# KevynUtopia/Frequency-Aware-Inverse-Consistent-OCTA-Super-Resolution

Hardware: AMD Instinct MI355X
Metric: train-step images/sec (G+D fwd+bwd) on 256x256 OCTA (higher is better)
Workload: dtype f32 (tensors and accumulators fp32; the convolutions' operands enter the matrix cores as f16x2 pairs: hi = f16(x 2^k), lo = f16(x 2^k - hi), k from the tensor's largest magnitude; 3 v_mfma_f32_32x32x16_f16 per product) on every map >= 24 wide with >= 16 channels; narrow maps, 1-channel stems / head

## Files before the change

frequency-aware-inverse-consistent-octa-super-resolution_amd/_lib.py:

```python
import ctypes
import os

import torch

_HERE = os.path.dirname(os.path.abspath(__file__))
LIB_PATH = os.environ.get("FAOCTASR_LIB") or os.path.join(_HERE, "libfaoctasr.so")

_P, _I, _L, _F = ctypes.c_void_p, ctypes.c_int, ctypes.c_long, ctypes.c_float
_SIG = {
    "version": (_I, ""),
    "last_error": (ctypes.c_char_p, ""),
    "last_route": (_I, ""),
    "conv_wpack_floats": (_L, "iiiiiiii"),
    "conv_pack_job": (_L, "p l i pp iiiiiiiii i i i"),
    "conv_pack_run": (_I, "p i l p"),
    "conv_pack_scales": (_I, "p i p"),
    "absmax_bits": (_I, "p l p p"),
    "conv_set_scales": (_I, "pp"),
    "conv_needs_scales": (_I, "i iiiiiiiii i i"),
    "out_absmax": (_I, "p"),
    "conv_set_workspace": (_I, "p l"),
    "conv_set_residual": (_I, "p"),
    "conv_wgrad_workspace_floats": (_L, "iiiii"),
    "conv_gather_workspace_floats": (_L, "i iiiiiiiii i i"),
    "conv2d_fwd": (_I, "pppp iiiiiiiii i i f p i i p"),
    "conv2d_dgrad": (_I, "ppp iiiiiiiii p i i p"),
    "conv2d_wgrad": (_I, "ppp iiiiiiiii i i i p"),
    "conv_transpose2d_fwd": (_I, "pppp iiiiiiiii i i f p i i p"),
    "conv_transpose2d_dgrad": (_I, "ppp iiiiiiiii i p i i p"),
    "conv_transpose2d_wgrad": (_I, "ppp iiiiiiiii i i i p"),
    "reflect_pad_bwd": (_I, "pp iiii p"),
    "channel_sum": (_I, "pp iii i p"),
    "bn_workspace_floats": (_L, "i"),
    "batchnorm_train_fwd": (_I, "ppppppppp iii ff i f p p"),
    "batchnorm_train_bwd": (_I, "ppppppppppp iii i f i p p"),
    "batchnorm_eval_fwd": (_I, "pppppp iii f i f p"),
    "batchnorm_eval_bwd": (_I, "ppppp iii f i f p"),
    "instancenorm_fwd": (_I, "pppppp iii f i f p p"),
    "instancenorm_bwd": (_I, "pppppppppp iii i f p p"),
    "act_fwd": (_I, "pp l i f p"),
    "act_bwd": (_I, "ppp l i f p"),
    "cat2_act_fwd": (_I, "ppp iiii i f p"),
    "cat2_act_bwd": (_I, "pppp iiii i f p"),
    "axpby": (_I, "ppp l ff p"),
    "haar_dwt2d_fwd": (_I, "ppp l ii p"),
    "haar_dwt2d_bwd": (_I, "ppp l ii p"),
    "haar_dfront_fwd": (_I, "pp iii i p"),
    "haar_dfront_bwd": (_I, "pp iii i p"),
    "sgemm_batched": (_I, "ppp iii iii lll i p"),
    "freq_mix_fwd": (_I, "ppppp l p"),
    "freq_mix_bwd": (_I, "pppppppp l p"),
    "ssim_fwd": (_I, "ppp iiii p"),
    "ssim_bwd": (_I, "ppp i f pp iiii p"),
    "dft_tables": (_I, "p i p"),
    "phase_loss_workspace_floats": (_L, "iiii"),
    "phase_loss_fwd": (_I, "pppp f ppp iiii p"),
    "phase_loss_bwd": (_I, "ppp f ppp iiii p"),
    "ffl_workspace_floats": (_L, "iiii"),
    "ffl_fwd": (_I, "pppp f ii ppp iiii p"),
    "ffl_bwd": (_I, "pppp f i ppp iiii p"),
    "mi_workspace_floats": (_L, "iiii i"),
    "mi_fwd": (_I, "pp ppp iiii i ffff ii p"),
    "mi_bwd": (_I, "ppp p pp iiii i fff i p"),
    "tv_loss_workspace_floats": (_L, "iiii"),
    "tv_loss_fwd": (_I, "ppp iiii f p"),
    "tv_loss_bwd": (_I, "ppp iiii f p"),
    "dwt2d_analysis": (_I, "ppp l ii ppi ppi i p"),
    "dwt2d_synthesis": (_I, "ppp l iiii ppi ppi i p"),
    "dwt1d_fused_max": (_L, ""),
    "dwt1d_analysis": (_I, "p lll pp l i p i pp i i i p"),
    "dwt1d_synthesis": (_I, "p lll pp l p i i pp i i i p"),
    "swt2d_analysis": (_I, "p l p l ii ppi ppi i i f p"),
    "swt2d_adjoint": (_I, "pp l p l i l ii ppi ppi i i f p"),
    "dtcwt_fwd_j1": (_I, "p lll pp llllll i l iii pi pi i p"),
    "dtcwt_fwd_j2": (_I, "p lll pp llllll i l iii pppp i p"),
    "dtcwt_inv_j1": (_I, "p lll p llllll p l iii pi pi i p"),
    "dtcwt_inv_j2": (_I, "p lll p llllll p l iii pppp i p"),
    "scat_fwd_j1": (_I, "p lll p ll i p lll p i ff l iii pi pi i p"),
    "scat_fwd_j2": (_I, "p lll p ll p lll p i ff l iii pppp i p"),
    "scat_bwd_j1": (_I, "p ll i p lll p p l iii pi pi i p"),
    "scat_bwd_j2": (_I, "p ll p lll p p l iii pppp i p"),
    "dtcwt_fwd_j1_bp": (_I, "p lll pp llllll i l iii pi pi pi i p"),
    "dtcwt_fwd_j2_bp": (_I, "p lll pp llllll i l iii pppppp i p"),
    "dtcwt_inv_j1_bp": (_I, "p lll p llllll p l iii pi pi pi i p"),
    "dtcwt_inv_j2_bp": (_I, "p lll p llllll p l iii pppppp i p"),
    "scat_fwd_j1_bp": (_I, "p lll p ll i p lll p i ff l iii pi pi pi i p"),
    "scat_fwd_j2_bp": (_I, "p lll p ll p lll p i ff l iii pppppp i p"),
    "scat_bwd_j1_bp": (_I, "p ll i p lll p p l iii pi pi pi i p"),
    "scat_bwd_j2_bp": (_I, "p ll p lll p p l iii pppppp i p"),
    "dtcwt_loss_workspace_floats": (_L, "l iii i"),
    "dtcwt_loss_fwd_j1": (_I, "p lll p lll pp pp p ff l iii pi pi i p"),
    "dtcwt_loss_fwd_j2": (_I, "p lll p lll pp pp p ff l iii pppp i p"),
    "dtcwt_loss_final": (_I, "p pp i p p"),
    "cwssim_workspace_floats": (_L, "l iii"),
    "cwssim_index": (_I, "pp pp p l iii f p"),
    "cwssim_grad": (_I, "pp pp pp p l l iii p"),
    "cwssim_final": (_I, "p l l iii pp p"),
    "msssim_workspace_floats": (_L, "l iii"),
    "msssim_scale_fwd": (_I, "pp pp p l iii i ff p"),
    "msssim_final": (_I, "p ll iii p i ppp p"),
    "msssim_scale_bwd": (_I, "pp p p i pp pp ll iii i ff p"),
    "loss_workspace_floats": (_L, ""),
    "loss_fwd": (_I, "ppp l i f p p"),
    "loss_bwd": (_I, "pppp l i f i p"),
    "mean_mix_fwd": (_I, "ppp iii ff p"),
    "mean_mix_bwd": (_I, "ppp iii ff p"),
    "adamw_step": (_I, "pppp l fffff i f p"),
    "adamw_step_dev": (_I, "pppp l p p"),
    "prep_crop_resize": (_I, "pppp iiiii ff p"),
    "fill": (_I, "p l f p"),
    "circulant_lowpass": (_I, "p i f p"),
    "eval_workspace_bytes": (_L, "ii"),
    "eval_metrics": (_I, "pppp iii f i p"),
    "bn_fold": (_I, "pppppp f pp i l i l p"),
# ... 92 lines not shown
```

frequency-aware-inverse-consistent-octa-super-resolution_amd/build.py:

```python
import os
import subprocess
from concurrent.futures import ThreadPoolExecutor

HERE = os.path.dirname(os.path.abspath(__file__))
ROOT = os.path.dirname(HERE)
SOURCES = ["igemm.hip", "igemm_patch.hip", "igemm_bf16x3.hip", "igemm_wino.hip", "igemm_nm.hip", "igemm_nm_x2.hip", "wgrad_patch.hip", "wgrad_s1.hip", "wgrad_x3.hip", "conv_m1.hip", "pointwise.hip", "norm.hip", "sgemm.hip",
           "ssim.hip", "spectral.hip", "mi.hip", "tv.hip", "dwt.hip", "dwt1d.hip", "swt.hip", "dtcwt.hip", "scat.hip", "dtcwt_loss.hip", "cwssim.hip", "msssim.hip", "eval.hip", "comm.hip", "conv_pack.hip", "conv_stem.hip"]
HEADERS = [os.path.join(HERE, "csrc", "common.h"), os.path.join(HERE, "csrc", "igemm_geom.h"), os.path.join(HERE, "csrc", "pack_bodies.h"), os.path.join(HERE, "csrc", "split16.h"), os.path.join(HERE, "csrc", "dtcwt_dev.h"),
           os.path.join(HERE, "csrc", "filterbank_dev.h"), os.path.join(HERE, "csrc", "ssim_window.h"),
           os.path.join(ROOT, "include", "faoctasr.h")]
FILE_FLAGS = {"ssim.hip": ["-fno-slp-vectorize"]}
LIB = os.path.join(HERE, "libfaoctasr.so")
OBJ_DIR = os.path.join(ROOT, "build", "obj")


def _flags():
    extra = os.environ.get("FAOCTASR_HIPCC_FLAGS", "").split()
    return ["-O3", "--offload-arch=gfx950", "-fPIC", "-std=c++17"] + extra + ["-I" + os.path.join(ROOT, "include"), "-I" + os.path.join(HERE, "csrc")]


def _stale(target, deps):
    if not os.path.exists(target):
        return True
    t = os.path.getmtime(target)
    return any(os.path.getmtime(d) > t for d in deps if os.path.exists(d))


def needs_build():
    srcs = [os.path.join(HERE, "csrc", s) for s in SOURCES]
    return _stale(LIB, srcs + HEADERS)


def build(force=False, verbose=False):
    hipcc = os.environ.get("HIPCC", "/opt/rocm/bin/hipcc")
    os.makedirs(OBJ_DIR, exist_ok=True)
    tag = "_".join(os.environ.get("FAOCTASR_HIPCC_FLAGS", "").split()).replace("/", "_").replace("=", "-")
    jobs, objs = [], []
    for s in SOURCES:
        src = os.path.join(HERE, "csrc", s)
        obj = os.path.join(OBJ_DIR, s + (("." + tag) if tag else "") + ".o")
        objs.append(obj)
        if force or _stale(obj, [src] + HEADERS):
            jobs.append((s, [hipcc] + _flags() + FILE_FLAGS.get(s, []) + ["-c", src, "-o", obj]))

    def run(job):
        name, cmd = job
        r = subprocess.run(cmd, stdout=subprocess.PIPE, stderr=subprocess.STDOUT, text=True)
        if r.returncode != 0:
            raise RuntimeError("hipcc failed on %s:\n%s\n%s" % (name, " ".join(cmd), r.stdout))
        return name

    if jobs:
        with ThreadPoolExecutor(max_workers=min(6, len(jobs))) as ex:
            done = list(ex.map(run, jobs))
        if verbose:
            print("compiled for gfx950:", " ".join(done))
    if jobs or force or _stale(LIB, objs):
        cmd = [hipcc, "--offload-arch=gfx950", "-fPIC", "-shared"] + objs + ["-ldl", "-o", LIB + ".tmp"]
        r = subprocess.run(cmd, stdout=subprocess.PIPE, stderr=subprocess.STDOUT, text=True)
        if r.returncode != 0:
            raise RuntimeError("link failed:\n%s\n%s" % (" ".join(cmd), r.stdout))
        os.replace(LIB + ".tmp", LIB)
        if verbose:
            print("linked", LIB)
    elif verbose:
        print("up to date:", LIB)
    return LIB


if __name__ == "__main__":
    import sys
    print(build(force="--force" in sys.argv, verbose=True))
```

frequency-aware-inverse-consistent-octa-super-resolution_amd/csrc/pointwise.hip:

```cpp
#include <mutex>
#include <unordered_map>
#include "common.h"
#include "split16.h"

namespace faoctasr {

thread_local char g_err[512] = "";
char* err_buf() { return g_err; }
int get_route();
int fail(int code, const char* fmt, ...) {
    va_list ap;
    va_start(ap, fmt);
    vsnprintf(g_err, sizeof(g_err), fmt, ap);
    va_end(ap);
    return code;
}

thread_local int g_route = 0;
thread_local unsigned* g_out_absmax = nullptr;
unsigned* take_out_absmax() {
    unsigned* p = g_out_absmax;
    g_out_absmax = nullptr;
    return p;
}
// ... 378 lines not shown
    constexpr float A = -0.75f;
    const float x0 = t + 1.f, x1 = t, x2 = 1.f - t, x3 = 2.f - t;
    c[0] = ((A * x0 - 5.f * A) * x0 + 8.f * A) * x0 - 4.f * A;
    c[1] = ((A + 2.f) * x1 - (A + 3.f)) * x1 * x1 + 1.f;
    c[2] = ((A + 2.f) * x2 - (A + 3.f)) * x2 * x2 + 1.f;
    c[3] = ((A * x3 - 5.f * A) * x3 + 8.f * A) * x3 - 4.f * A;
}

__global__ void prep_crop_resize_kernel(const unsigned char* __restrict__ img, const int* __restrict__ tops, const int* __restrict__ lefts,
                                        float* __restrict__ out, int N, int H, int W, int crop, int osz, float mean, float inv_std) {
    const long total = (long)N * osz * osz;
    const float scale = (float)crop / (float)osz;
    for (long i = (long)blockIdx.x * blockDim.x + threadIdx.x; i < total; i += (long)gridDim.x * blockDim.x) {
        const int ox = (int)(i % osz), oy = (int)((i / osz) % osz), n = (int)(i / ((long)osz * osz));
        const unsigned char* src = img + (long)n * H * W + (long)tops[n] * W + lefts[n];
        float v;
        if (osz == crop) {
            v = (float)src[(long)oy * W + ox] / 255.f;
        } else {
            const float sy = ((float)oy + 0.5f) * scale - 0.5f, sx = ((float)ox + 0.5f) * scale - 0.5f;
            const float fy = floorf(sy), fx = floorf(sx);
            float cy[4], cx[4];
            cubic_coeffs(sy - fy, cy);
            cubic_coeffs(sx - fx, cx);
            const int iy = (int)fy, ix = (int)fx;
            v = 0.f;
#pragma unroll
            for (int a = 0; a < 4; ++a) {
                int yy = iy - 1 + a;
                yy = yy < 0 ? 0 : (yy > crop - 1 ? crop - 1 : yy);
                float row = 0.f;
#pragma unroll
                for (int b = 0; b < 4; ++b) {
                    int xx = ix - 1 + b;
                    xx = xx < 0 ? 0 : (xx > crop - 1 ? crop - 1 : xx);
                    row += cx[b] * ((float)src[(long)yy * W + xx] / 255.f);
                }
                v += cy[a] * row;
            }
        }
        out[i] = (v - mean) * inv_std;
    }
}

__global__ __launch_bounds__(256) void absmax_bits_kernel(const float* __restrict__ x, long n, unsigned* __restrict__ slot) {
    typedef unsigned u32x4v __attribute__((ext_vector_type(4)));
    unsigned mx = 0;
    const long n4 = (reinterpret_cast<unsigned long>(x) & 15) ? 0 : n >> 2;
    const u32x4v* x4 = reinterpret_cast<const u32x4v*>(x);
    const long stride = (long)gridDim.x * 256;
    long i = (long)blockIdx.x * 256 + threadIdx.x;
    for (; i + 3 * stride < n4; i += 4 * stride) {
        const u32x4v v0 = x4[i], v1 = x4[i + stride], v2 = x4[i + 2 * stride], v3 = x4[i + 3 * stride];
#pragma unroll
        for (int j = 0; j < 4; ++j) {
            const unsigned a = v0[j] & 0x7fffffffu, b = v1[j] & 0x7fffffffu, c = v2[j] & 0x7fffffffu, d = v3[j] & 0x7fffffffu;
            const unsigned ab = a > b ? a : b, cd = c > d ? c : d;
            const unsigned m4 = ab > cd ? ab : cd;
            mx = m4 > mx ? m4 : mx;
        }
    }
    for (; i < n4; i += stride) {
        const u32x4v v = x4[i];
#pragma unroll
        for (int j = 0; j < 4; ++j) {
            const unsigned b = v[j] & 0x7fffffffu;
            mx = b > mx ? b : mx;
        }
    }
    for (long k = (n4 << 2) + (long)blockIdx.x * 256 + threadIdx.x; k < n; k += stride) {
        const unsigned b = __builtin_bit_cast(unsigned, x[k]) & 0x7fffffffu;
        mx = b > mx ? b : mx;
    }
    __shared__ unsigned red[4];
    absmax_publish_block(mx, slot, red);
}

}

using namespace faoctasr;

extern "C" {

int faoctasr_version(void) { return 440; }
const char* faoctasr_last_error(void) { return err_buf(); }
int faoctasr_last_route(void) { return faoctasr::get_route(); }

int faoctasr_batchnorm_eval_fwd(const float* x, const float* gamma, const float* beta, const float* running_mean, const float* running_var,
                                float* y, int N, int C, int HW, float eps, int act, float slope, faoctasr_stream_t stream) {
    if (!x || !y || !running_mean || !running_var) return fail(FAOCTASR_EINVAL, "batchnorm_eval_fwd: null pointer");
    const long total = (long)N * C * HW;
    if (total <= 0) return FAOCTASR_OK;
    hipLaunchKernelGGL(bn_eval_fwd_kernel, dim3(grid_for(total, 1024)), dim3(256), 0, (hipStream_t)stream, x, gamma, beta, running_mean,
                       running_var, y, C, HW, total, eps, act, slope);
    return check_launch("bn_eval_fwd");
}

int faoctasr_batchnorm_eval_bwd(const float* dy, const float* y, const float* gamma, const float* running_var, float* dx, int N, int C, int HW,
                                float eps, int act, float slope, faoctasr_stream_t stream) {
    if (!dy || !dx || !running_var) return fail(FAOCTASR_EINVAL, "batchnorm_eval_bwd: null pointer");
    if (act != FAOCTASR_ACT_NONE && !y) return fail(FAOCTASR_EINVAL, "batchnorm_eval_bwd: activation mask needs the forward output");
    const long total = (long)N * C * HW;
    if (total <= 0) return FAOCTASR_OK;
    hipLaunchKernelGGL(bn_eval_bwd_kernel, dim3(grid_for(total, 1024)), dim3(256), 0, (hipStream_t)stream, dy, y, gamma, running_var, dx, C,
                       HW, total, eps, act, slope);
    return check_launch("bn_eval_bwd");
}

int faoctasr_act_fwd(const float* x, float* y, long n, int act, float slope, faoctasr_stream_t stream) {
    if (!x || !y) return fail(FAOCTASR_EINVAL, "act_fwd: null pointer");
    if (n <= 0) return FAOCTASR_OK;
    hipLaunchKernelGGL(act_fwd_kernel, dim3(grid_for(n, 1024)), dim3(256), 0, (hipStream_t)stream, x, y, n, act, slope);
    return check_launch("act_fwd");
}

int faoctasr_act_bwd(const float* dy, const float* y, float* dx, long n, int act, float slope, faoctasr_stream_t stream) {
    if (!dy || !y || !dx) return fail(FAOCTASR_EINVAL, "act_bwd: null pointer");
    if (n <= 0) return FAOCTASR_OK;
    hipLaunchKernelGGL(act_bwd_kernel, dim3(grid_for(n, 1024)), dim3(256), 0, (hipStream_t)stream, dy, y, dx, n, act, slope);
    return check_launch("act_bwd");
}

int faoctasr_cat2_act_fwd(const float* a, const float* b, float* y, int N, int Ca, int Cb, int HW, int act, float slope,
                          faoctasr_stream_t stream) {
    if (!a || !b || !y) return fail(FAOCTASR_EINVAL, "cat2_act_fwd: null pointer");
    const long tot = (long)N * (Ca + Cb) * HW;
    if (tot <= 0) return FAOCTASR_OK;
    hipLaunchKernelGGL(cat2_act_fwd_kernel, dim3(grid_for(tot, 256)), dim3(256), 0, (hipStream_t)stream, a, b, y, N, (long)Ca * HW,
                       (long)Cb * HW, act, slope, faoctasr::take_out_absmax());
    return check_launch("cat2_act_fwd");
}

int faoctasr_cat2_act_bwd(const float* dy, const float* y, float* da, float* db, int N, int Ca, int Cb, int HW, int act, float slope,
                          faoctasr_stream_t stream) {
    if (!dy) return fail(FAOCTASR_EINVAL, "cat2_act_bwd: null pointer");
    if (act != FAOCTASR_ACT_NONE && !y) return fail(FAOCTASR_EINVAL, "cat2_act_bwd: mask needs y");
    const long tot = (long)N * (Ca + Cb) * HW;
    if (tot <= 0) return FAOCTASR_OK;
    hipLaunchKernelGGL(cat2_act_bwd_kernel, dim3(grid_for(tot, 256)), dim3(256), 0, (hipStream_t)stream, dy, y, da, db, N,
                       (long)Ca * HW, (long)Cb * HW, act, slope);
    return check_launch("cat2_act_bwd");
}

int faoctasr_axpby(const float* a, const float* b, float* y, long n, float alpha, float beta, faoctasr_stream_t stream) {
    if (!a || !b || !y) return fail(FAOCTASR_EINVAL, "axpby: null pointer");
    if (n <= 0) return FAOCTASR_OK;
    hipLaunchKernelGGL(axpby_kernel, dim3(grid_for(n, 256)), dim3(256), 0, (hipStream_t)stream, a, b, y, n, alpha, beta);
    return check_launch("axpby");
}

int faoctasr_fill(float* p, long n, float value, faoctasr_stream_t stream) {
    if (!p) return fail(FAOCTASR_EINVAL, "fill: null pointer");
    if (n <= 0) return FAOCTASR_OK;
    hipLaunchKernelGGL(fill_kernel, dim3(grid_for(n, 256)), dim3(256), 0, (hipStream_t)stream, p, n, value);
    return check_launch("fill");
}

int faoctasr_channel_sum(const float* dy, float* db, int N, int C, int HW, int accumulate, faoctasr_stream_t stream) {
    if (!dy || !db) return fail(FAOCTASR_EINVAL, "channel_sum: null pointer");
    if (C <= 0) return FAOCTASR_OK;
    hipStream_t st = (hipStream_t)stream;
    if (!accumulate && hipMemsetAsync(db, 0, sizeof(float) * C, st) != hipSuccess) return fail(FAOCTASR_EHIP, "channel_sum: memset failed");
    const long L = (long)N * HW;
    long S = (1024 + C - 1) / C;
    const long maxs = (L + 4095) / 4096;
    S = S < maxs ? S : maxs;
    S = S < 1 ? 1 : S;
// ... 149 lines not shown
```

frequency-aware-inverse-consistent-octa-super-resolution_amd/ops.py:

```python
import contextlib
import ctypes
import math

import torch
from torch.autograd import Function

from . import _lib
from ._lib import call, ptr, stream_ptr

ACT_NONE, ACT_RELU, ACT_LRELU, ACT_TANH = 0, 1, 2, 3
_ACT = {None: 0, "none": 0, "relu": 1, "lrelu": 2, "tanh": 3}

direct_grad = True
fuse_residual_grad = True


def act_code(a):
    return a if isinstance(a, int) else _ACT[a]


def _c(t):
    if not t.is_cuda:
        raise _lib.KernelError("operand lives on %s: the HIP operators have no CPU/eager fallback" % t.device)
    return t if t.is_contiguous() else t.contiguous()


import weakref

weight_epoch = 0
use_wpack = True
conv_precision = 0
PRECISIONS = {"f32": 0, "f32_direct": 1, "bf16x3": 2, "f16x2": 3}
reproducible_forward = False
NO_SPLIT_K = 0x100
_wpack_cache = {}
pack_misses = 0


def invalidate_weight_cache():
    global weight_epoch
    weight_epoch += 1


_scale_arenas = {}
SCALE_ARENA_SLOTS = 1024
SLOT_WORDS = 128


def reset_scale_arenas():
    _scale_arenas.clear()


absmax_log = None


def _new_slot(device):
    sid = stream_ptr()
    ent = _scale_arenas.get(sid)
    if ent is None or ent[1] >= SCALE_ARENA_SLOTS or ent[0].device != device:
        ent = _scale_arenas[sid] = [torch.zeros(SCALE_ARENA_SLOTS * SLOT_WORDS, dtype=torch.float32, device=device), 0]
    i = ent[1]
    ent[1] = i + 1
    return ent[0][i * SLOT_WORDS:(i + 1) * SLOT_WORDS]


def absmax_slot(t):
    sid = stream_ptr()
    c = getattr(t, "_fa_absmax", None)
    if c is not None and c[1] == t._version and c[2] == sid:
        return c[0]
    slot = _new_slot(t.device)
    call("absmax_bits", ptr(t), t.numel(), ptr(slot), sid)
    t._fa_absmax = (slot, t._version, sid)
    if absmax_log is not None:
        why = "no tag" if c is None else ("version" if c[1] != t._version else "stream")
        key = (tuple(t.shape), why)
        absmax_log[key] = absmax_log.get(key, 0) + 1
    return slot


def _producer_slot(x, C, H, W):
    if conv_precision != 3 or C < 16 or (H * W) & 3:
        return None
    return _new_slot(x.device)


def _producer_call(name, args, slot):
    if slot is not None:
        call("out_absmax", ptr(slot))
    call(name, *args)


def _tag_absmax(t, slot):
    if slot is not None:
        t._fa_absmax = (slot, t._version, stream_ptr())


# ... 143 lines not shown
                cur = torch.cuda.current_stream()
                if cur.cuda_stream == aside.cuda_stream:
                    aside = None
                else:
                    aside.wait_stream(cur)
            with torch.cuda.stream(aside) if aside is not None else contextlib.nullcontext():
                if self.precision == 3:
                    call("conv_pack_scales", ptr(self.table), self.njobs, stream_ptr())
                call("conv_pack_run", ptr(self.table), self.njobs, self.nblocks, stream_ptr())
                if aside is not None:
                    event, ev_stream = aside.record_event(), aside.cuda_stream
        for e, w in live:
            e.ver = _ver(w)
            e.event, e.ev_stream = event, ev_stream
        return True


wgrad_stream = None
_wgrad_keep = {}
wait_guard = None


wgrad_defer = False
_deferred = []


def end_wgrad():
    global wgrad_stream
    side, held = wgrad_stream, list(_deferred)
    del _deferred[:]
    wgrad_stream = None
    if held and side is not None:
        seen = {side.cuda_stream}
        for _, _, src in held + [(None, None, torch.cuda.current_stream())]:
            if src.cuda_stream not in seen:
                seen.add(src.cuda_stream)
                if wait_guard is not None:
                    wait_guard(side.cuda_stream, src.cuda_stream)
                side.wait_stream(src)
        with torch.cuda.stream(side):
            for fn, operands, _ in held:
                fn(side.cuda_stream)
                _wgrad_keep.setdefault(side.cuda_stream, []).append(operands)
    elif held:
        for fn, _, _ in held:
            fn(stream_ptr())


def _enqueue_wgrad(fn, *operands):
    side = wgrad_stream
    if side is None:
        fn(stream_ptr())
        return
    if wgrad_defer:
        _deferred.append((fn, operands, torch.cuda.current_stream()))
        return
    cur = torch.cuda.current_stream()
    if cur.cuda_stream != side.cuda_stream:
        if wait_guard is not None:
            wait_guard(side.cuda_stream, cur.cuda_stream)
        side.wait_stream(cur)
    with torch.cuda.stream(side):
        fn(side.cuda_stream)
    _wgrad_keep.setdefault(side.cuda_stream, []).append(operands)


def join_wgrad_stream(side):
    if side is not None:
        cur = torch.cuda.current_stream()
        if cur.cuda_stream != side.cuda_stream:
            if wait_guard is not None:
                wait_guard(cur.cuda_stream, side.cuda_stream)
            cur.wait_stream(side)
        _wgrad_keep.pop(side.cuda_stream, None)


def _grad_target(p):
    g = p.grad
    if direct_grad and g is not None and g.is_contiguous() and g.dtype == torch.float32:
        return g
    return None


class _Conv2d(Function):
    @staticmethod
    def forward(ctx, x, w, bias, stride, pad, reflect, act, slope, link=None):
        ctx.link = link
        x, w = _c(x), _c(w)
        N, C, IH, IW = x.shape
        M, Cw, KH, KW = w.shape
        if Cw != C:
            raise _lib.KernelError("conv2d: input has %d channels, weight expects %d" % (C, Cw))
        OH, OW = (IH + 2 * pad - KH) // stride + 1, (IW + 2 * pad - KW) // stride + 1
        if OH <= 0 or OW <= 0:
            raise RuntimeError("Calculated padded input size per channel: (%d x %d). Kernel size: (%d x %d). "
                               "Kernel size can't be greater than actual input size" % (IH + 2 * pad, IW + 2 * pad, KH, KW))
        y = torch.empty((N, M, OH, OW), dtype=torch.float32, device=x.device)
        wp, wst, ent = _wpack(w, 0, (N, C, IH, IW, M, KH, KW, stride, pad), reflect)
        sx = absmax_slot(x) if _needs_scales(0, (N, C, IH, IW, M, KH, KW, stride, pad), reflect) else None
        _gather_workspace(x.device, 0, (N, C, IH, IW, M, KH, KW, stride, pad), reflect)
        _conv_call("conv2d_fwd", (ptr(x), ptr(w), ptr(bias), ptr(y), N, C, IH, IW, M, KH, KW, stride, pad, reflect, act, slope, ptr(wp), wst,
                                  conv_precision | (NO_SPLIT_K if reproducible_forward else 0), stream_ptr()), sx)
        _packed(ent, wst)
        ctx.sx = sx
        ctx.save_for_backward(x, w, y if act else None)
        ctx.w_ref, ctx.b_ref = w, bias
        ctx.cfg = (stride, pad, reflect, act, slope)
        return y

    @staticmethod
    def backward(ctx, dy):
        x, w, y = ctx.saved_tensors
        stride, pad, reflect, act, slope = ctx.cfg
        dy = _c(dy)
        st = stream_ptr()
        N, C, IH, IW = x.shape
        M, _, KH, KW = w.shape
        if act:
            g = torch.empty_like(dy)
            call("act_bwd", ptr(dy), ptr(y), ptr(g), dy.numel(), act, slope, st)
            dy = g
        dx = dw = db = None
        dg_dims = (N, C, IH + 2 * pad, IW + 2 * pad, M, KH, KW, stride, 0) if reflect else (N, C, IH, IW, M, KH, KW, stride, pad)
        need_d = _needs_scales(1, dg_dims) if ctx.needs_input_grad[0] else 0
        need_w = _needs_scales(4, (N, C, IH, IW, M, KH, KW, stride, pad), reflect) if ctx.needs_input_grad[1] else 0
        sdy = absmax_slot(dy) if (need_d or need_w) else None
        res = ctx.link.pop("dres", None) if ctx.link is not None else None
        if res is not None and not ctx.needs_input_grad[0]:
            raise _lib.KernelError("a residual link left a skip gradient for a convolution whose input needs no gradient")
        if ctx.needs_input_grad[0]:
            sd = sdy if need_d else None
            if res is not None:
                res = _c(res)
            if reflect:
                dxp = torch.empty((N, C, IH + 2 * pad, IW + 2 * pad), dtype=torch.float32, device=x.device)
                wp, wst, ent = _wpack(ctx.w_ref, 1, (N, C, IH + 2 * pad, IW + 2 * pad, M, KH, KW, stride, 0))
                _gather_workspace(x.device, 1, dg_dims)
                _conv_call("conv2d_dgrad", (ptr(dy), ptr(w), ptr(dxp), N, C, IH + 2 * pad, IW + 2 * pad, M, KH, KW, stride, 0, ptr(wp), wst,
                                            conv_precision, st), sd)
                _packed(ent, wst)
                dx = torch.empty_like(x)
                call("reflect_pad_bwd", ptr(dxp), ptr(dx), N * C, IH, IW, pad, st)
                if res is not None:
                    call("axpby", ptr(dx), ptr(res), ptr(dx), dx.numel(), 1.0, 1.0, st)
            else:
                dx = torch.empty_like(x)
                wp, wst, ent = _wpack(ctx.w_ref, 1, (N, C, IH, IW, M, KH, KW, stride, pad))
                _gather_workspace(x.device, 1, dg_dims)
                _conv_call("conv2d_dgrad", (ptr(dy), ptr(w), ptr(dx), N, C, IH, IW, M, KH, KW, stride, pad, ptr(wp), wst, conv_precision, st), sd, None, res)
                _packed(ent, wst)
        if ctx.needs_input_grad[1]:
            tgt = _grad_target(ctx.w_ref)
            if tgt is None:
                dw = torch.empty_like(w)
            prec = conv_precision
            sx = None
            if need_w:
                sx = ctx.sx if ctx.sx is not None else absmax_slot(x)
            elif prec == 3:
                prec = 0
            sdw = sdy if need_w else None

            def wgrad(s, out, accumulate):
                _wgrad_workspace(x.device, C, M, KH, KW, stride, prec)
                _conv_call("conv2d_wgrad", (ptr(x), ptr(dy), ptr(out), N, C, IH, IW, M, KH, KW, stride, pad, reflect, accumulate, prec, s), sx, sdw)
            if tgt is not None:
                _enqueue_wgrad(lambda s: wgrad(s, tgt, 1), x, dy, sx, sdw)
            else:
                wgrad(st, dw, 0)
        if ctx.b_ref is not None and ctx.needs_input_grad[2]:
            tb = _grad_target(ctx.b_ref)
            if tb is not None:
                _enqueue_wgrad(lambda s: call("channel_sum", ptr(dy), ptr(tb), N, M, dy.shape[2] * dy.shape[3], 1, s), dy)
            else:
                db = torch.empty(M, dtype=torch.float32, device=x.device)
                call("channel_sum", ptr(dy), ptr(db), N, M, dy.shape[2] * dy.shape[3], 0, st)
        return dx, dw, db, None, None, None, None, None, None


def conv2d(x, w, bias=None, stride=1, pad=0, reflect=False, act=None, slope=0.2, link=None):
    return _Conv2d.apply(x, w, bias, int(stride), int(pad), 1 if reflect else 0, act_code(act), float(slope), link)


class _ConvTranspose2d(Function):
    @staticmethod
    def forward(ctx, x, w, bias, stride, pad, out_pad, act, slope):
        x, w = _c(x), _c(w)
        N, C, IH, IW = x.shape
        Cw, M, KH, KW = w.shape
        if Cw != C:
            raise _lib.KernelError("conv_transpose2d: input has %d channels, weight expects %d" % (C, Cw))
        OH, OW = (IH - 1) * stride - 2 * pad + KH + out_pad, (IW - 1) * stride - 2 * pad + KW + out_pad
        y = torch.empty((N, M, OH, OW), dtype=torch.float32, device=x.device)
        wp, wst, ent = _wpack(w, 2, (N, C, IH, IW, M, KH, KW, stride, pad), 0, out_pad)
        sx = absmax_slot(x) if _needs_scales(2, (N, C, IH, IW, M, KH, KW, stride, pad), 0, out_pad) else None
        ctx.sx = sx
        _gather_workspace(x.device, 2, (N, C, IH, IW, M, KH, KW, stride, pad), 0, out_pad)
        _conv_call("conv_transpose2d_fwd", (ptr(x), ptr(w), ptr(bias), ptr(y), N, C, IH, IW, M, KH, KW, stride, pad, out_pad, act, slope,
                                            ptr(wp), wst, conv_precision | (NO_SPLIT_K if reproducible_forward else 0), stream_ptr()), sx)
        _packed(ent, wst)
        ctx.save_for_backward(x, w, y if act else None)
        ctx.w_ref, ctx.b_ref = w, bias
        ctx.cfg = (stride, pad, out_pad, act, slope)
        return y

    @staticmethod
    def backward(ctx, dy):
        x, w, y = ctx.saved_tensors
        stride, pad, out_pad, act, slope = ctx.cfg
        dy = _c(dy)
        st = stream_ptr()
        N, C, IH, IW = x.shape
        _, M, KH, KW = w.shape
        if act:
            g = torch.empty_like(dy)
            call("act_bwd", ptr(dy), ptr(y), ptr(g), dy.numel(), act, slope, st)
            dy = g
# ... 1901 lines not shown
```

include/faoctasr.h:

```cpp
#ifndef FAOCTASR_H
#define FAOCTASR_H

#ifdef __cplusplus
extern "C" {
#endif

typedef void* faoctasr_stream_t;

enum { FAOCTASR_ACT_NONE = 0, FAOCTASR_ACT_RELU = 1, FAOCTASR_ACT_LRELU = 2, FAOCTASR_ACT_TANH = 3 };
enum { FAOCTASR_OK = 0, FAOCTASR_EINVAL = -1, FAOCTASR_EUNSUPPORTED = -2, FAOCTASR_EHIP = -3 };

int faoctasr_version(void);
const char* faoctasr_last_error(void);
int faoctasr_last_route(void);

int faoctasr_conv2d_fwd(const float* x, const float* w, const float* bias, float* y,
                        int N, int C, int IH, int IW, int M, int KH, int KW, int stride, int pad,
                        int reflect, int act, float slope, float* wpack, int wpack_state, int precision,
                        faoctasr_stream_t stream);
#define FAOCTASR_CONV_NO_SPLIT_K 0x100
long faoctasr_conv_wpack_floats(int kind, int C, int M, int KH, int KW, int stride, int pad, int precision);
#define FAOCTASR_PACK_JOB_BYTES 1024
long faoctasr_conv_pack_job(void* job_host, long block_base, int kind, const float* w, float* wpack,
                            int N, int C, int IH, int IW, int M, int KH, int KW, int stride, int pad,
                            int reflect, int out_pad, int precision);
int faoctasr_conv_pack_run(const void* jobs_dev, int njobs, long nblocks, faoctasr_stream_t stream);
int faoctasr_conv_pack_scales(const void* jobs_dev, int njobs, faoctasr_stream_t stream);
#define FAOCTASR_ABSMAX_SLOT_WORDS 128
int faoctasr_absmax_bits(const float* x, long n, unsigned* slot, faoctasr_stream_t stream);
int faoctasr_out_absmax(unsigned* slot);
int faoctasr_conv_set_scales(const unsigned* slot_a, const unsigned* slot_b);
int faoctasr_conv_needs_scales(int kind, int N, int C, int IH, int IW, int M, int KH, int KW, int stride, int pad,
                               int reflect, int out_pad);
int faoctasr_conv_set_workspace(float* workspace, long nfloats);
long faoctasr_conv_gather_workspace_floats(int kind, int N, int C, int IH, int IW, int M, int KH, int KW, int stride, int pad,
                                           int reflect, int out_pad);
int faoctasr_conv_set_residual(const float* residual);
long faoctasr_conv_wgrad_workspace_floats(int C, int M, int KH, int KW, int stride);
int faoctasr_conv2d_dgrad(const float* dy, const float* w, float* dx,
                          int N, int C, int IH, int IW, int M, int KH, int KW, int stride, int pad,
                          float* wpack, int wpack_state, int precision, faoctasr_stream_t stream);
int faoctasr_conv2d_wgrad(const float* x, const float* dy, float* dw,
                          int N, int C, int IH, int IW, int M, int KH, int KW, int stride, int pad,
                          int reflect, int accumulate, int precision, faoctasr_stream_t stream);
int faoctasr_conv_transpose2d_fwd(const float* x, const float* w, const float* bias, float* y,
                                  int N, int C, int IH, int IW, int M, int KH, int KW, int stride, int pad,
                                  int out_pad, int act, float slope, float* wpack, int wpack_state, int precision,
                                  faoctasr_stream_t stream);
int faoctasr_conv_transpose2d_dgrad(const float* dy, const float* w, float* dx,
                                    int N, int C, int IH, int IW, int M, int KH, int KW, int stride, int pad,
                                    int out_pad, float* wpack, int wpack_state, int precision, faoctasr_stream_t stream);
int faoctasr_conv_transpose2d_wgrad(const float* x, const float* dy, float* dw,
                                    int N, int C, int IH, int IW, int M, int KH, int KW, int stride, int pad,
                                    int out_pad, int accumulate, int precision, faoctasr_stream_t stream);
int faoctasr_reflect_pad_bwd(const float* dxp, float* dx, int NC, int H, int W, int p, faoctasr_stream_t stream);
int faoctasr_channel_sum(const float* dy, float* db, int N, int C, int HW, int accumulate, faoctasr_stream_t stream);

long faoctasr_bn_workspace_floats(int C);
int faoctasr_batchnorm_train_fwd(const float* x, const float* gamma, const float* beta, const float* residual,
                                 float* y, float* save_mean, float* save_invstd,
                                 float* running_mean, float* running_var,
                                 int N, int C, int HW, float eps, float momentum, int act, float slope,
                                 float* workspace, faoctasr_stream_t stream);
int faoctasr_batchnorm_train_bwd(const float* x, const float* dy, const float* y, const float* gamma, const float* beta,
                                 const float* save_mean, const float* save_invstd,
                                 float* dx, float* dgamma, float* dbeta, float* dres,
                                 int N, int C, int HW, int act, float slope, int accumulate_affine,
                                 float* workspace, faoctasr_stream_t stream);
int faoctasr_batchnorm_eval_fwd(const float* x, const float* gamma, const float* beta, const float* running_mean,
                                const float* running_var, float* y, int N, int C, int HW, float eps, int act, float slope,
                                faoctasr_stream_t stream);
int faoctasr_batchnorm_eval_bwd(const float* dy, const float* y, const float* gamma, const float* running_var, float* dx,
                                int N, int C, int HW, float eps, int act, float slope, faoctasr_stream_t stream);
int faoctasr_instancenorm_fwd(const float* x, const float* gamma, const float* beta, float* y,
                              float* save_mean, float* save_invstd, int N, int C, int HW, float eps,
                              int act, float slope, float* workspace, faoctasr_stream_t stream);
int faoctasr_instancenorm_bwd(const float* x, const float* dy, const float* y, const float* gamma, const float* beta,
                              const float* save_mean, const float* save_invstd, float* dx,
                              float* dgamma, float* dbeta, int N, int C, int HW, int act, float slope,
                              float* workspace, faoctasr_stream_t stream);

int faoctasr_act_fwd(const float* x, float* y, long n, int act, float slope, faoctasr_stream_t stream);
int faoctasr_act_bwd(const float* dy, const float* y, float* dx, long n, int act, float slope, faoctasr_stream_t stream);
int faoctasr_cat2_act_fwd(const float* a, const float* b, float* y, int N, int Ca, int Cb, int HW,
                          int act, float slope, faoctasr_stream_t stream);
int faoctasr_cat2_act_bwd(const float* dy, const float* y, float* da, float* db, int N, int Ca, int Cb, int HW,
                          int act, float slope, faoctasr_stream_t stream);
int faoctasr_axpby(const float* a, const float* b, float* y, long n, float alpha, float beta, faoctasr_stream_t stream);

int faoctasr_haar_dwt2d_fwd(const float* x, float* ll, float* hi, long NC, int H, int W, faoctasr_stream_t stream);
int faoctasr_haar_dwt2d_bwd(const float* dll, const float* dhi, float* dx, long NC, int H, int W, faoctasr_stream_t stream);
int faoctasr_haar_dfront_fwd(const float* x, float* y, int N, int H, int W, int mode, faoctasr_stream_t stream);
int faoctasr_haar_dfront_bwd(const float* dy, float* dx, int N, int H, int W, int mode, faoctasr_stream_t stream);

int faoctasr_sgemm_batched(const float* A, const float* B, float* C, int M, int N, int K,
                           int lda, int ldb, int ldc, long strideA, long strideB, long strideC, int batch,
                           faoctasr_stream_t stream);
int faoctasr_circulant_lowpass(float* out, int n, float radius, faoctasr_stream_t stream);
int faoctasr_freq_mix_fwd(const float* x, const float* low_hp, const float* low_lp, float* hf, float* lf,
                          long n, faoctasr_stream_t stream);
int faoctasr_freq_mix_bwd(const float* x, const float* low_hp, const float* low_lp, const float* g_hf, const float* g_lf,
                          float* s_hp, float* s_lp, float* dx_direct, long n, faoctasr_stream_t stream);

int faoctasr_ssim_fwd(const float* a, const float* b, float* sums, int N, int C, int H, int W, faoctasr_stream_t stream);
int faoctasr_ssim_bwd(const float* a, const float* b, const float* g, int gN, float gscale, float* da, float* db,
                      int N, int C, int H, int W, faoctasr_stream_t stream);

int faoctasr_dft_tables(float* out, int n, faoctasr_stream_t stream);
long faoctasr_phase_loss_workspace_floats(int N, int C, int H, int W);
int faoctasr_phase_loss_fwd(const float* x, const float* y, const float* tabH, const float* tabW, float radius,
                            float* loss_per_sample, float* loss_mean, float* workspace, int N, int C, int H, int W,
                            faoctasr_stream_t stream);
int faoctasr_phase_loss_bwd(const float* g, const float* tabH, const float* tabW, float radius, float* dx, float* dy,
                            float* workspace, int N, int C, int H, int W, faoctasr_stream_t stream);

long faoctasr_ffl_workspace_floats(int N, int C, int H, int W);
int faoctasr_ffl_fwd(const float* x, const float* y, const float* tabH, const float* tabW, float alpha, int log_matrix,
                     int batch_matrix, float* loss, float* planes, float* workspace, int N, int C, int H, int W,
                     faoctasr_stream_t stream);
int faoctasr_ffl_bwd(const float* g, const float* planes, const float* tabH, const float* tabW, float alpha, int log_matrix,
                     float* dx, float* dy, float* workspace, int N, int C, int H, int W, faoctasr_stream_t stream);

long faoctasr_mi_workspace_floats(int N, int C, int H, int W, int bins);
int faoctasr_mi_fwd(const float* x, const float* y, float* out, float* table, float* workspace, int N, int C, int H, int W,
                    int bins, float lo, float hi, float sigma_ratio, float eps, int normalized, int per_image,
                    faoctasr_stream_t stream);
int faoctasr_mi_bwd(const float* g, const float* x, const float* y, const float* table, float* dx, float* dy, int N, int C,
                    int H, int W, int bins, float lo, float hi, float sigma_ratio, int per_image, faoctasr_stream_t stream);

long faoctasr_tv_loss_workspace_floats(int B, int C, int H, int W);
int faoctasr_tv_loss_fwd(const float* x, float* out, float* workspace, int B, int C, int H, int W, float weight,
                         faoctasr_stream_t stream);
int faoctasr_tv_loss_bwd(const float* x, const float* g, float* dx, int B, int C, int H, int W, float weight,
                         faoctasr_stream_t stream);

int faoctasr_dwt2d_analysis(const float* x, float* ll, float* hi, long NC, int H, int W, const float* lo_h, const float* hi_h,
                            int L_h, const float* lo_w, const float* hi_w, int L_w, int mode, faoctasr_stream_t stream);
int faoctasr_dwt2d_synthesis(const float* ll, const float* hi, float* y, long NC, int nh, int nw, int out_h, int out_w,
// ... 146 lines not shown
```

Baseline: 136.9.

## Compute reflect-padded conv dgrad on unpadded map plus border correction kernel

For 7x7 stride-1 reflect-padded convolutions, the input gradient is now computed by a zero-padded dgrad directly on the unpadded map, followed by a new kernel that folds the mirrored border contributions back into the edge rows and columns. This removes the padded-size dgrad output allocation and the separate reflect-pad backward pass. The cost is two extra border-correction launches. These are small FP32 FMA kernels that re-read dy edge rows and the weights for every output-channel chunk.

```diff
diff --git a/frequency-aware-inverse-consistent-octa-super-resolution_amd/_lib.py b/frequency-aware-inverse-consistent-octa-super-resolution_amd/_lib.py
--- a/frequency-aware-inverse-consistent-octa-super-resolution_amd/_lib.py
+++ b/frequency-aware-inverse-consistent-octa-super-resolution_amd/_lib.py
@@ -30,6 +30,8 @@
     "conv_transpose2d_dgrad": (_I, "ppp iiiiiiiii i p i i p"),
     "conv_transpose2d_wgrad": (_I, "ppp iiiiiiiii i i i p"),
     "reflect_pad_bwd": (_I, "pp iiii p"),
+    "reflect_dgrad_border_ok": (_I, "iiiiii"),
+    "reflect_dgrad_border": (_I, "ppp iiiiiii p"),
     "channel_sum": (_I, "pp iii i p"),
     "bn_workspace_floats": (_L, "i"),
     "batchnorm_train_fwd": (_I, "ppppppppp iii ff i f p p"),
diff --git a/frequency-aware-inverse-consistent-octa-super-resolution_amd/build.py b/frequency-aware-inverse-consistent-octa-super-resolution_amd/build.py
--- a/frequency-aware-inverse-consistent-octa-super-resolution_amd/build.py
+++ b/frequency-aware-inverse-consistent-octa-super-resolution_amd/build.py
@@ -5,11 +5,11 @@
 HERE = os.path.dirname(os.path.abspath(__file__))
 ROOT = os.path.dirname(HERE)
 SOURCES = ["igemm.hip", "igemm_patch.hip", "igemm_bf16x3.hip", "igemm_wino.hip", "igemm_nm.hip", "igemm_nm_x2.hip", "wgrad_patch.hip", "wgrad_s1.hip", "wgrad_x3.hip", "conv_m1.hip", "pointwise.hip", "norm.hip", "sgemm.hip",
-           "ssim.hip", "spectral.hip", "mi.hip", "tv.hip", "dwt.hip", "dwt1d.hip", "swt.hip", "dtcwt.hip", "scat.hip", "dtcwt_loss.hip", "cwssim.hip", "msssim.hip", "eval.hip", "comm.hip", "conv_pack.hip", "conv_stem.hip"]
+           "ssim.hip", "spectral.hip", "mi.hip", "tv.hip", "dwt.hip", "dwt1d.hip", "swt.hip", "dtcwt.hip", "scat.hip", "dtcwt_loss.hip", "cwssim.hip", "msssim.hip", "eval.hip", "comm.hip", "conv_pack.hip", "conv_stem.hip", "reflect_dgrad.hip"]
 HEADERS = [os.path.join(HERE, "csrc", "common.h"), os.path.join(HERE, "csrc", "igemm_geom.h"), os.path.join(HERE, "csrc", "pack_bodies.h"), os.path.join(HERE, "csrc", "split16.h"), os.path.join(HERE, "csrc", "dtcwt_dev.h"),
            os.path.join(HERE, "csrc", "filterbank_dev.h"), os.path.join(HERE, "csrc", "ssim_window.h"),
            os.path.join(ROOT, "include", "faoctasr.h")]
-FILE_FLAGS = {"ssim.hip": ["-fno-slp-vectorize"]}
+FILE_FLAGS = {"ssim.hip": ["-fno-slp-vectorize"], "reflect_dgrad.hip": ["-fno-slp-vectorize"]}
 LIB = os.path.join(HERE, "libfaoctasr.so")
 OBJ_DIR = os.path.join(ROOT, "build", "obj")
 
diff --git a/frequency-aware-inverse-consistent-octa-super-resolution_amd/csrc/pointwise.hip b/frequency-aware-inverse-consistent-octa-super-resolution_amd/csrc/pointwise.hip
--- a/frequency-aware-inverse-consistent-octa-super-resolution_amd/csrc/pointwise.hip
+++ b/frequency-aware-inverse-consistent-octa-super-resolution_amd/csrc/pointwise.hip
@@ -484,7 +484,7 @@
 
 extern "C" {
 
-int faoctasr_version(void) { return 440; }
+int faoctasr_version(void) { return 450; }
 const char* faoctasr_last_error(void) { return err_buf(); }
 int faoctasr_last_route(void) { return faoctasr::get_route(); }
 
diff --git a/frequency-aware-inverse-consistent-octa-super-resolution_amd/csrc/reflect_dgrad.hip b/frequency-aware-inverse-consistent-octa-super-resolution_amd/csrc/reflect_dgrad.hip
--- /dev/null
+++ b/frequency-aware-inverse-consistent-octa-super-resolution_amd/csrc/reflect_dgrad.hip
@@ -0,0 +1,238 @@
+#include "common.h"
+
+namespace faoctasr {
+
+constexpr int RD_WAVES = 8;
+constexpr int RD_CC = 8;
+
+template <int P>
+struct RdCfg {
+    static constexpr int K = 2 * P + 1;
+    static_assert(K <= 8, "a kernel row is staged as 8 floats");
+    static constexpr int SPAN = 64 + 2 * P;
+    static constexpr int SROW = (SPAN + 4) & ~3;
+    static constexpr int WC = K * 8;
+    static constexpr int WF = RD_CC * WC;
+    static constexpr int REGION = WF + P * SROW;
+    static constexpr int NWL = (RD_CC * K * K + 63) / 64, NSL = (SPAN + 63) / 64;
+    static constexpr int RED = RD_WAVES * P * RD_CC * 64;
+    static_assert(RD_WAVES * REGION <= RED, "the staging regions live in the reduction buffer");
+};
+
+__device__ __forceinline__ void rd_wave_sync() {
+    __builtin_amdgcn_fence(__ATOMIC_RELEASE, "wavefront");
+    __builtin_amdgcn_wave_barrier();
+    __builtin_amdgcn_fence(__ATOMIC_ACQUIRE, "wavefront");
+}
+
+template <int P>
+__device__ __forceinline__ void rd_weights(const float* wl, int ci, float (&wr)[2 * P + 1][8]) {
+    using Cfg = RdCfg<P>;
+#pragma unroll
+    for (int r = 0; r < Cfg::K; ++r)
+#pragma unroll
+        for (int h = 0; h < 2; ++h) {
+            const float4 q = *reinterpret_cast<const float4*>(wl + ci * Cfg::WC + r * 8 + h * 4);
+            wr[r][h * 4 + 0] = q.x; wr[r][h * 4 + 1] = q.y; wr[r][h * 4 + 2] = q.z; wr[r][h * 4 + 3] = q.w;
+        }
+}
+
+template <int P, bool VERT, int SIDE>
+__device__ __forceinline__ void rd_fma(const float* wl, const float (&e)[P][2 * P + 1], float (&acc)[P][RD_CC]) {
+    constexpr int K = 2 * P + 1;
+    float wr[2][K][8];
+    rd_weights<P>(wl, 0, wr[0]);
+#pragma unroll
+    for (int ci = 0; ci < RD_CC; ++ci) {
+        if (ci + 1 < RD_CC) rd_weights<P>(wl, ci + 1, wr[(ci + 1) & 1]);
+#pragma unroll
+        for (int o = 0; o < P; ++o) {
+#pragma unroll
+            for (int rho = 0; rho < P; ++rho) {
+                if (SIDE == 0 ? rho > o : rho > P - 1 - o) continue;
+                const int ta = SIDE == 0 ? o - rho : P + 1 + o + rho;
+#pragma unroll
+                for (int t = 0; t < K; ++t) acc[o][ci] = fmaf(VERT ? wr[ci & 1][t][ta] : wr[ci & 1][ta][t], e[rho][t], acc[o][ci]);
+            }
+        }
+    }
+}
+
+template <int P, bool VERT>
+struct RdLane {
+    using Cfg = RdCfg<P>;
+    static constexpr int K = Cfg::K;
+    int wsrc[Cfg::NWL], wdst[Cfg::NWL];
+    int ssrc[Cfg::NSL], sdst[Cfg::NSL];
+    unsigned sok;
+    int a, lane, mbase;
+    unsigned okm;
+    bool valid, any_mirror;
+
+    __device__ __forceinline__ void init(int a0, int lane_, int L, int sL, int nc) {
+        lane = lane_; a = a0 + lane;
+        valid = a < L;
+#pragma unroll
+        for (int k = 0; k < Cfg::NWL; ++k) {
+            const int f = lane + 64 * k, last = nc * K * K - 1;
+            wsrc[k] = f < last ? f : last;
+            const int c = f / (K * K), r = f % (K * K);
+            wdst[k] = f < RD_CC * K * K ? c * Cfg::WC + (r / K) * 8 + r % K : 7;
+        }
+        sok = 0u;
+#pragma unroll
+        for (int k = 0; k < Cfg::NSL; ++k) {
+            const int idx = lane + 64 * k, pos = a0 - P + idx;
+            if (idx < Cfg::SPAN && pos >= 0 && pos < L) sok |= 1u << k;
+            ssrc[k] = (pos < 0 ? 0 : (pos > L - 1 ? L - 1 : pos)) * sL;
+            sdst[k] = idx < Cfg::SPAN ? idx : Cfg::SROW - 1;
+        }
+        const bool ml = !VERT && valid && a >= 1 && a <= P;
+        const bool mr = !VERT && valid && !ml && a >= L - 1 - P && a <= L - 2;
+        const int qm = ml ? P - a : 2 * (L - 1) - a + P;
+        okm = 0u;
+#pragma unroll
+        for (int t = 0; t < K; ++t)
+            if ((ml || mr) && qm - t >= 0 && qm - t < L) okm |= 1u << t;
+        mbase = (ml || mr) ? qm - (a0 - P) : K - 1;
+        any_mirror = !VERT && __any(ml || mr);
+    }
+
+    struct Regs { float w[Cfg::NWL], s[P][Cfg::NSL]; };
+    __device__ __forceinline__ void fetch(const float* __restrict__ plane, const float* __restrict__ wm, int side, int A, int sA, Regs& r) const {
+#pragma unroll
+        for (int k = 0; k < Cfg::NWL; ++k) r.w[k] = wm[wsrc[k]];
+#pragma unroll
+        for (int rho = 0; rho < P; ++rho) {
+            const float* __restrict__ row = plane + (long)(side ? A - 1 - rho : rho) * sA;
+#pragma unroll
+            for (int k = 0; k < Cfg::NSL; ++k) r.s[rho][k] = row[ssrc[k]];
+        }
+    }
+
+    __device__ __forceinline__ void stage(const Regs& r, float* wl, float* sl, float (&e)[P][K]) const {
+        rd_wave_sync();
+#pragma unroll
+        for (int k = 0; k < Cfg::NWL; ++k) wl[wdst[k]] = r.w[k];
+#pragma unroll
+        for (int rho = 0; rho < P; ++rho)
+#pragma unroll
+            for (int k = 0; k < Cfg::NSL; ++k) sl[rho * Cfg::SROW + sdst[k]] = ((sok >> k) & 1u) ? r.s[rho][k] : 0.f;
+        rd_wave_sync();
+#pragma unroll
+        for (int rho = 0; rho < P; ++rho)
+#pragma unroll
+            for (int t = 0; t < K; ++t) e[rho][t] = sl[rho * Cfg::SROW + lane + 2 * P - t];
+        if constexpr (!VERT) {
+            if (any_mirror) {
+#pragma unroll
+                for (int t = 0; t < K; ++t) {
+                    int idx = mbase - t;
+                    idx = idx < 0 ? 0 : (idx > Cfg::SPAN - 1 ? Cfg::SPAN - 1 : idx);
+#pragma unroll
+                    for (int rho = 0; rho < P; ++rho) {
+                        const float v = sl[rho * Cfg::SROW + idx];
+                        e[rho][t] += ((okm >> t) & 1u) ? v : 0.f;
+                    }
+                }
+            }
+        }
+    }
+};
+
+template <int P, bool VERT, int SIDE>
+__device__ __forceinline__ void rd_body(const float* __restrict__ dy, const float* __restrict__ w, const RdLane<P, VERT>& ln, int n, int c0, int C,
+                                        int M, long HW, int A, int sA, int wv, float* wl, float* sl, float (&acc)[P][RD_CC]) {
+    constexpr int K = 2 * P + 1;
+    float e[P][K];
+    typename RdLane<P, VERT>::Regs r;
+    if (wv < M) ln.fetch(dy + ((long)n * M + wv) * HW, w + ((long)wv * C + c0) * (K * K), SIDE, A, sA, r);
+#pragma unroll 1
+    for (int m = wv; m < M; m += RD_WAVES) {
+        ln.stage(r, wl, sl, e);
+        const int mn = m + RD_WAVES < M ? m + RD_WAVES : m;
+        ln.fetch(dy + ((long)n * M + mn) * HW, w + ((long)mn * C + c0) * (K * K), SIDE, A, sA, r);
+        __builtin_amdgcn_sched_barrier(0);
+        rd_fma<P, VERT, SIDE>(wl, e, acc);
+    }
+}
+
+template <int P, bool VERT>
+__global__ __launch_bounds__(64 * RD_WAVES) void reflect_dgrad_border_kernel(const float* __restrict__ dy, const float* __restrict__ w,
+                                                                             float* __restrict__ dx, int C, int H, int W, int M, int nseg,
+                                                                             int nchunk) {
+    using Cfg = RdCfg<P>;
+    __shared__ __attribute__((aligned(16))) float lds[Cfg::RED];
+    unsigned bi = blockIdx.x;
+    const int seg = (int)(bi % (unsigned)nseg); bi /= (unsigned)nseg;
+    const int c0 = (int)(bi % (unsigned)nchunk) * RD_CC; bi /= (unsigned)nchunk;
+    const int side = (int)(bi & 1u), n = (int)(bi >> 1);
+    const int lane = threadIdx.x & 63;
+    const int wv = __builtin_amdgcn_readfirstlane((int)(threadIdx.x >> 6));
+    const int L = VERT ? H : W, A = VERT ? W : H, sL = VERT ? W : 1, sA = VERT ? 1 : W;
+    const long HW = (long)H * W;
+
+    RdLane<P, VERT> ln;
+    ln.init(seg * 64, lane, L, sL, C - c0 < RD_CC ? C - c0 : RD_CC);
+    float* wl = lds + wv * Cfg::REGION;
+    float* sl = wl + Cfg::WF;
+
+    float acc[P][RD_CC];
+#pragma unroll
+    for (int o = 0; o < P; ++o)
+#pragma unroll
+        for (int ci = 0; ci < RD_CC; ++ci) acc[o][ci] = 0.f;
+    if (side == 0) rd_body<P, VERT, 0>(dy, w, ln, n, c0, C, M, HW, A, sA, wv, wl, sl, acc);
+    else rd_body<P, VERT, 1>(dy, w, ln, n, c0, C, M, HW, A, sA, wv, wl, sl, acc);
+
+    __syncthreads();
+#pragma unroll
+    for (int o = 0; o < P; ++o)
+#pragma unroll
+        for (int ci = 0; ci < RD_CC; ++ci) lds[(wv * P * RD_CC + o * RD_CC + ci) * 64 + lane] = acc[o][ci];
+    __syncthreads();
+    for (int line = wv; line < P * RD_CC; line += RD_WAVES) {
+        const int o = line / RD_CC, c = c0 + line % RD_CC;
+        float s = lds[line * 64 + lane];
+#pragma unroll
+        for (int v = 1; v < RD_WAVES; ++v) s += lds[(v * P * RD_CC + line) * 64 + lane];
+        if (ln.valid && c < C) {
+            const int tgt = side ? A - 2 - o : P - o;
+            float* q = dx + ((long)n * C + c) * HW + (long)tgt * sA + (long)ln.a * sL;
+            *q += s;
+        }
+    }
+}
+
+template <int P>
+static int rd_launch(const float* dy, const float* w, float* dx, int N, int C, int H, int W, int M, hipStream_t s) {
+    const int nchunk = (C + RD_CC - 1) / RD_CC;
+    const int nseg_h = (W + 63) / 64, nseg_v = (H + 63) / 64;
+    const long bh = (long)N * 2 * nchunk * nseg_h, bv = (long)N * 2 * nchunk * nseg_v;
+    if (bh > 0x7fffffffL || bv > 0x7fffffffL) return fail(FAOCTASR_EINVAL, "reflect_dgrad_border: tensor too large");
+    hipLaunchKernelGGL((reflect_dgrad_border_kernel<P, false>), dim3((unsigned)bh), dim3(64 * RD_WAVES), 0, s, dy, w, dx, C, H, W, M, nseg_h, nchunk);
+    hipLaunchKernelGGL((reflect_dgrad_border_kernel<P, true>), dim3((unsigned)bv), dim3(64 * RD_WAVES), 0, s, dy, w, dx, C, H, W, M, nseg_v, nchunk);
+    return check_launch("reflect_dgrad_border");
+}
+
+}
+
+using namespace faoctasr;
+
+extern "C" {
+
+int faoctasr_reflect_dgrad_border_ok(int IH, int IW, int KH, int KW, int stride, int pad) {
+    return stride == 1 && pad == 3 && KH == 2 * pad + 1 && KW == 2 * pad + 1 && IH >= 2 * pad + 2 && IW >= 2 * pad + 2;
+}
+
+int faoctasr_reflect_dgrad_border(const float* dy, const float* w, float* dx, int N, int C, int IH, int IW, int M, int K, int pad,
+                                  faoctasr_stream_t stream) {
+    if (!dy || !w || !dx) return fail(FAOCTASR_EINVAL, "reflect_dgrad_border: null pointer");
+    if (N < 0 || C <= 0 || M <= 0) return fail(FAOCTASR_EINVAL, "reflect_dgrad_border: bad shape");
+    if (!faoctasr_reflect_dgrad_border_ok(IH, IW, K, K, 1, pad))
+        return fail(FAOCTASR_EUNSUPPORTED, "reflect_dgrad_border: needs K = 7, pad = 3 and a map of at least 8 x 8 (got K %d, pad %d, %d x %d)", K, pad, IH, IW);
+    if (N == 0) return FAOCTASR_OK;
+    return rd_launch<3>(dy, w, dx, N, C, IH, IW, M, (hipStream_t)stream);
+}
+
+}
diff --git a/frequency-aware-inverse-consistent-octa-super-resolution_amd/ops.py b/frequency-aware-inverse-consistent-octa-super-resolution_amd/ops.py
--- a/frequency-aware-inverse-consistent-octa-super-resolution_amd/ops.py
+++ b/frequency-aware-inverse-consistent-octa-super-resolution_amd/ops.py
@@ -1,6 +1,7 @@
 import contextlib
 import ctypes
 import math
+import os
 
 import torch
 from torch.autograd import Function
@@ -8,11 +9,24 @@
 from . import _lib
 from ._lib import call, ptr, stream_ptr
 
+
+def _env_choice(name, choices, default):
+    v = os.environ.get(name)
+    if v is None or v == "":
+        return default
+    if v not in choices:
+        raise ValueError("%s=%r: expected one of %s" % (name, v, sorted(choices)))
+    return choices[v]
+
+
 ACT_NONE, ACT_RELU, ACT_LRELU, ACT_TANH = 0, 1, 2, 3
 _ACT = {None: 0, "none": 0, "relu": 1, "lrelu": 2, "tanh": 3}
 
 direct_grad = True
 fuse_residual_grad = True
+
+
+reflect_dgrad_border = _env_choice("FAOCTASR_REFLECT_DGRAD", {"border": True, "padded": False}, True)
 
 
 def act_code(a):
@@ -322,6 +336,32 @@
     return None
 
 
+_border_ok_cache = {}
+
+
+def _border_ok(IH, IW, KH, KW, stride, pad):
+    key = (IH, IW, KH, KW, stride, pad)
+    r = _border_ok_cache.get(key)
+    if r is None:
+        r = _border_ok_cache[key] = bool(_lib.load().faoctasr_reflect_dgrad_border_ok(*key))
+    return r
+
+
+def reflect_dgrad_border_reference(dy, w, pad):
+    H, W = dy.shape[-2:]
+    full = torch.nn.functional.conv_transpose2d(dy, w)
+    full[..., pad:pad + H, pad:pad + W] = 0
+
+    def fold(t, dim, n):
+        i = torch.arange(n + 2 * pad, device=t.device) - pad
+        i = torch.where(i < 0, -i, torch.where(i > n - 1, 2 * (n - 1) - i, i))
+        shape = list(t.shape)
+        shape[dim] = n
+        return torch.zeros(shape, dtype=t.dtype, device=t.device).index_add_(dim, i, t)
+
+    return fold(fold(full, -2, H), -1, W)
+
+
 class _Conv2d(Function):
     @staticmethod
     def forward(ctx, x, w, bias, stride, pad, reflect, act, slope, link=None):
@@ -361,7 +401,11 @@
             call("act_bwd", ptr(dy), ptr(y), ptr(g), dy.numel(), act, slope, st)
             dy = g
         dx = dw = db = None
-        dg_dims = (N, C, IH + 2 * pad, IW + 2 * pad, M, KH, KW, stride, 0) if reflect else (N, C, IH, IW, M, KH, KW, stride, pad)
+        border = bool(reflect and reflect_dgrad_border and ctx.needs_input_grad[0] and _border_ok(IH, IW, KH, KW, stride, pad))
+        if reflect and not border:
+            dg_dims = (N, C, IH + 2 * pad, IW + 2 * pad, M, KH, KW, stride, 0)
+        else:
+            dg_dims = (N, C, IH, IW, M, KH, KW, stride, pad)
         need_d = _needs_scales(1, dg_dims) if ctx.needs_input_grad[0] else 0
         need_w = _needs_scales(4, (N, C, IH, IW, M, KH, KW, stride, pad), reflect) if ctx.needs_input_grad[1] else 0
         sdy = absmax_slot(dy) if (need_d or need_w) else None
@@ -372,7 +416,14 @@
             sd = sdy if need_d else None
             if res is not None:
                 res = _c(res)
-            if reflect:
+            if border:
+                dx = torch.empty_like(x)
+                wp, wst, ent = _wpack(ctx.w_ref, 1, dg_dims)
+                _gather_workspace(x.device, 1, dg_dims)
+                _conv_call("conv2d_dgrad", (ptr(dy), ptr(w), ptr(dx), N, C, IH, IW, M, KH, KW, stride, pad, ptr(wp), wst, conv_precision, st), sd, None, res)
+                _packed(ent, wst)
+                call("reflect_dgrad_border", ptr(dy), ptr(w), ptr(dx), N, C, IH, IW, M, KH, pad, st)
+            elif reflect:
                 dxp = torch.empty((N, C, IH + 2 * pad, IW + 2 * pad), dtype=torch.float32, device=x.device)
                 wp, wst, ent = _wpack(ctx.w_ref, 1, (N, C, IH + 2 * pad, IW + 2 * pad, M, KH, KW, stride, 0))
                 _gather_workspace(x.device, 1, dg_dims)
diff --git a/include/faoctasr.h b/include/faoctasr.h
--- a/include/faoctasr.h
+++ b/include/faoctasr.h
@@ -54,6 +54,9 @@
                                     int N, int C, int IH, int IW, int M, int KH, int KW, int stride, int pad,
                                     int out_pad, int accumulate, int precision, faoctasr_stream_t stream);
 int faoctasr_reflect_pad_bwd(const float* dxp, float* dx, int NC, int H, int W, int p, faoctasr_stream_t stream);
+int faoctasr_reflect_dgrad_border_ok(int IH, int IW, int KH, int KW, int stride, int pad);
+int faoctasr_reflect_dgrad_border(const float* dy, const float* w, float* dx,
+                                  int N, int C, int IH, int IW, int M, int K, int pad, faoctasr_stream_t stream);
 int faoctasr_channel_sum(const float* dy, float* db, int N, int C, int HW, int accumulate, faoctasr_stream_t stream);
 
 long faoctasr_bn_workspace_floats(int C);
```

Result: no change. 137.5, median of 6 (+0.5%).
